# upkie/upkie

Hardware: AMD Instinct MI355X
Metric: env-steps/sec (batched Upkie-Pendulum, 200 Hz) (higher is better)
Workload: dtype f32

## Files before the change

### upkie_amd/csrc/dynamics.hpp

```cpp
#pragma once

#include <hip/hip_runtime.h>

#include "../../include/upkie_hip.h"

#define UPKIE_HD __host__ __device__ __forceinline__

namespace upkie {

UPKIE_HD float fast_rcp(float x) {
#if defined(__HIP_DEVICE_COMPILE__)
  return __builtin_amdgcn_rcpf(x);
#else
  return 1.f / x;
#endif
}
UPKIE_HD float fast_sqrt(float x) {
#if defined(__HIP_DEVICE_COMPILE__)
  return __builtin_amdgcn_sqrtf(x);
#else
  return sqrtf(x);
#endif
}
UPKIE_HD float fast_rsqrt(float x) {
// ... 128 lines not shown
  int enforce_joint_limits;
};

struct DevLimits {
  float lower[UPKIE_NJ];
  float upper[UPKIE_NJ];
  int bounded[UPKIE_NJ];
  int enforce;
};

struct Phys {
  V3 pos;
  float qw, qx, qy, qz;
  V3 linvel;
  V3 angvel;
  float q[UPKIE_NJ];
  float qd[UPKIE_NJ];
};

#if defined(__HIP_DEVICE_COMPILE__)
#define UPKIE_KEEP_IN_SGPR(x) asm volatile("" : "+s"(x))
#else
#define UPKIE_KEEP_IN_SGPR(x) (void)0
#endif

#if defined(__HIP_DEVICE_COMPILE__)
__device__ __forceinline__ void warm_kernel_arguments() {
  auto args = __builtin_amdgcn_kernarg_segment_ptr();
  int sink;
  asm volatile(
      "s_load_dword %0, %1, 0x0\n s_load_dword %0, %1, 0x40\n s_load_dword %0, %1, 0x80\n s_load_dword %0, %1, 0xc0\n"
      "s_load_dword %0, %1, 0x100\n s_load_dword %0, %1, 0x140\n s_load_dword %0, %1, 0x180\n s_load_dword %0, %1, 0x1c0\n"
      "s_load_dword %0, %1, 0x200\n s_load_dword %0, %1, 0x240\n s_load_dword %0, %1, 0x280\n s_load_dword %0, %1, 0x2c0\n"
      "s_load_dword %0, %1, 0x300\n s_load_dword %0, %1, 0x340\n s_load_dword %0, %1, 0x380\n s_load_dword %0, %1, 0x3c0\n"
      "s_load_dword %0, %1, 0x400\n s_load_dword %0, %1, 0x440\n s_load_dword %0, %1, 0x480\n s_load_dword %0, %1, 0x4c0\n"
      "s_waitcnt lgkmcnt(0)"
      : "=&s"(sink)
      : "s"(args)
      : "memory");
}
template <int BYTES, class Ptr>
__device__ __forceinline__ void warm_constant_block(Ptr block) {
  constexpr int LINES = (BYTES + 63) / 64;
  static_assert(LINES <= 24, "block larger than the unrolled touch sequence");
#define UPKIE_LINE(i) "n"(64 * ((i) < LINES ? (i) : LINES - 1))
  int sink;
  asm volatile(
      "s_load_dword %0, %1, %2\n s_load_dword %0, %1, %3\n s_load_dword %0, %1, %4\n s_load_dword %0, %1, %5\n"
      "s_load_dword %0, %1, %6\n s_load_dword %0, %1, %7\n s_load_dword %0, %1, %8\n s_load_dword %0, %1, %9\n"
      "s_load_dword %0, %1, %10\n s_load_dword %0, %1, %11\n s_load_dword %0, %1, %12\n s_load_dword %0, %1, %13\n"
      "s_load_dword %0, %1, %14\n s_load_dword %0, %1, %15\n s_load_dword %0, %1, %16\n s_load_dword %0, %1, %17\n"
      "s_load_dword %0, %1, %18\n s_load_dword %0, %1, %19\n s_load_dword %0, %1, %20\n s_load_dword %0, %1, %21\n"
      "s_load_dword %0, %1, %22\n s_load_dword %0, %1, %23\n s_load_dword %0, %1, %24\n s_load_dword %0, %1, %25\n"
      "s_waitcnt lgkmcnt(0)"
      : "=&s"(sink)
      : "s"(block), UPKIE_LINE(0), UPKIE_LINE(1), UPKIE_LINE(2), UPKIE_LINE(3), UPKIE_LINE(4), UPKIE_LINE(5), UPKIE_LINE(6), UPKIE_LINE(7),
        UPKIE_LINE(8), UPKIE_LINE(9), UPKIE_LINE(10), UPKIE_LINE(11), UPKIE_LINE(12), UPKIE_LINE(13), UPKIE_LINE(14), UPKIE_LINE(15),
        UPKIE_LINE(16), UPKIE_LINE(17), UPKIE_LINE(18), UPKIE_LINE(19), UPKIE_LINE(20), UPKIE_LINE(21), UPKIE_LINE(22), UPKIE_LINE(23)
      : "memory");
#undef UPKIE_LINE
}
#else
__device__ inline void warm_kernel_arguments() {}
template <int BYTES, class Ptr>
__device__ inline void warm_constant_block(Ptr) {}
#endif

struct BaseFrame {
  float r00, r01, r02, r10, r11, r12, r20, r21, r22;
  V3 vB, wB, nB;
};
UPKIE_HD BaseFrame base_frame(float qw, float qx, float qy, float qz, V3 linvel, V3 angvel) {
  BaseFrame f;
  f.r00 = 1.f - 2.f * (qy * qy + qz * qz); f.r01 = 2.f * (qx * qy - qz * qw); f.r02 = 2.f * (qw * qy + qx * qz);
  f.r10 = 2.f * (qx * qy + qz * qw); f.r11 = 1.f - 2.f * (qx * qx + qz * qz); f.r12 = 2.f * (qy * qz - qx * qw);
  f.r20 = 2.f * (qx * qz - qy * qw); f.r21 = 2.f * (qy * qz + qx * qw); f.r22 = 1.f - 2.f * (qx * qx + qy * qy);
  f.vB = v3(f.r00 * linvel.x + f.r10 * linvel.y + f.r20 * linvel.z, f.r01 * linvel.x + f.r11 * linvel.y + f.r21 * linvel.z,
            f.r02 * linvel.x + f.r12 * linvel.y + f.r22 * linvel.z);
  f.wB = v3(f.r00 * angvel.x + f.r10 * angvel.y + f.r20 * angvel.z, f.r01 * angvel.x + f.r11 * angvel.y + f.r21 * angvel.z,
            f.r02 * angvel.x + f.r12 * angvel.y + f.r22 * angvel.z);
  f.nB = v3(f.r20, f.r21, f.r22);
  return f;
}
UPKIE_HD void integrate_base(const BaseFrame& f, float n0, float n1, float n2, float n3, float n4, float n5, float h, V3& pos, float& qw,
                             float& qx, float& qy, float& qz, V3& linvel, V3& angvel) {
  linvel = v3(f.r00 * n0 + f.r01 * n1 + f.r02 * n2, f.r10 * n0 + f.r11 * n1 + f.r12 * n2, f.r20 * n0 + f.r21 * n1 + f.r22 * n2);
  angvel = v3(f.r00 * n3 + f.r01 * n4 + f.r02 * n5, f.r10 * n3 + f.r11 * n4 + f.r12 * n5, f.r20 * n3 + f.r21 * n4 + f.r22 * n5);
  pos = pos + h * linvel;
  const float wn = fast_sqrt(dot(angvel, angvel));
  const float half = 0.5f * h * wn;
  float ch, k;
  if (half < 0.5f) {
    const float x2 = half * half;
    k = 0.5f * h * (1.f + x2 * (-1.f / 6.f + x2 * (1.f / 120.f + x2 * (-1.f / 5040.f + x2 * (1.f / 362880.f)))));
    ch = 1.f + x2 * (-0.5f + x2 * (1.f / 24.f + x2 * (-1.f / 720.f + x2 * (1.f / 40320.f))));
  } else {
    float sh;
    sincosf(half, &sh, &ch);
    k = sh * fast_rcp(wn);
  }
  const float dw = ch, dx = k * angvel.x, dy = k * angvel.y, dz = k * angvel.z;
  const float nw = dw * qw - dx * qx - dy * qy - dz * qz;
  const float nx = dw * qx + dx * qw + dy * qz - dz * qy;
  const float ny = dw * qy - dx * qz + dy * qw + dz * qx;
  const float nz = dw * qz + dx * qy - dy * qx + dz * qw;
  const float inv = fast_rsqrt(nw * nw + nx * nx + ny * ny + nz * nz);
  qw = nw * inv; qx = nx * inv; qy = ny * inv; qz = nz * inv;
}

struct Ldl6 {
  float l10, l20, l21, l30, l31, l32, l40, l41, l42, l43, l50, l51, l52, l53, l54;
  float i0, i1, i2, i3, i4, i5;
};

UPKIE_HD void ldl6_factor(const float (&A)[21], Ldl6& f) {
  float d0 = A[0];
  f.i0 = fast_rcp(d0);
  float a10 = A[1], a20 = A[3], a30 = A[6], a40 = A[10], a50 = A[15];
  f.l10 = a10 * f.i0; f.l20 = a20 * f.i0; f.l30 = a30 * f.i0; f.l40 = a40 * f.i0; f.l50 = a50 * f.i0;
  float d1 = A[2] - f.l10 * a10;
  f.i1 = fast_rcp(d1);
  float a21 = A[4] - f.l20 * a10, a31 = A[7] - f.l30 * a10, a41 = A[11] - f.l40 * a10, a51 = A[16] - f.l50 * a10;
  f.l21 = a21 * f.i1; f.l31 = a31 * f.i1; f.l41 = a41 * f.i1; f.l51 = a51 * f.i1;
  float d2 = A[5] - f.l20 * a20 - f.l21 * a21;
  f.i2 = fast_rcp(d2);
  float a32 = A[8] - f.l30 * a20 - f.l31 * a21, a42 = A[12] - f.l40 * a20 - f.l41 * a21,
        a52 = A[17] - f.l50 * a20 - f.l51 * a21;
  f.l32 = a32 * f.i2; f.l42 = a42 * f.i2; f.l52 = a52 * f.i2;
  float d3 = A[9] - f.l30 * a30 - f.l31 * a31 - f.l32 * a32;
  f.i3 = fast_rcp(d3);
  float a43 = A[13] - f.l40 * a30 - f.l41 * a31 - f.l42 * a32,
        a53 = A[18] - f.l50 * a30 - f.l51 * a31 - f.l52 * a32;
  f.l43 = a43 * f.i3; f.l53 = a53 * f.i3;
  float d4 = A[14] - f.l40 * a40 - f.l41 * a41 - f.l42 * a42 - f.l43 * a43;
  f.i4 = fast_rcp(d4);
  float a54 = A[19] - f.l50 * a40 - f.l51 * a41 - f.l52 * a42 - f.l53 * a43;
  f.l54 = a54 * f.i4;
  float d5 = A[20] - f.l50 * a50 - f.l51 * a51 - f.l52 * a52 - f.l53 * a53 - f.l54 * a54;
  f.i5 = fast_rcp(d5);
}

UPKIE_HD void ldl6_solve(const Ldl6& f, float (&x)[6]) {
  x[1] -= f.l10 * x[0];
  x[2] -= f.l20 * x[0] + f.l21 * x[1];
  x[3] -= f.l30 * x[0] + f.l31 * x[1] + f.l32 * x[2];
  x[4] -= f.l40 * x[0] + f.l41 * x[1] + f.l42 * x[2] + f.l43 * x[3];
  x[5] -= f.l50 * x[0] + f.l51 * x[1] + f.l52 * x[2] + f.l53 * x[3] + f.l54 * x[4];
  x[0] *= f.i0; x[1] *= f.i1; x[2] *= f.i2; x[3] *= f.i3; x[4] *= f.i4; x[5] *= f.i5;
  x[4] -= f.l54 * x[5];
  x[3] -= f.l43 * x[4] + f.l53 * x[5];
  x[2] -= f.l32 * x[3] + f.l42 * x[4] + f.l52 * x[5];
  x[1] -= f.l21 * x[2] + f.l31 * x[3] + f.l41 * x[4] + f.l51 * x[5];
  x[0] -= f.l10 * x[1] + f.l20 * x[2] + f.l30 * x[3] + f.l40 * x[4] + f.l50 * x[5];
}

struct Leg {
  V3 o[3];
  float F[3][6];
  float Hinv[6];
  float D[6][3];
  float bias[3];
  float sgn[3];
};

struct Composite {
  float m;
  V3 h;
  S3 I;
};

struct BodyInertials {
  float m[UPKIE_NB];
  float c[UPKIE_NB][3];
  float I[UPKIE_NB][6];
};
// ... 1353 lines not shown
```

### upkie_amd/csrc/octet.hpp

```cpp
#pragma once

#if !defined(__HIP_DEVICE_COMPILE__)
struct OctHostLane {
  int lane;
  float* slots;
  void (*barrier)(void*);
  void* arg;
};
inline thread_local OctHostLane* g_oct_lane = nullptr;
inline float oct_host_get(float x, int src) {
  OctHostLane* L = g_oct_lane;
  L->slots[L->lane] = x;
  L->barrier(L->arg);
  const float r = L->slots[src];
  L->barrier(L->arg);
  return r;
}
#endif

template <int S0, int S1, int S2, int S3>
UPKIE_HD float oct_qperm(float x) {
#if defined(__HIP_DEVICE_COMPILE__)
  return __builtin_bit_cast(float, __builtin_amdgcn_update_dpp(0, __builtin_bit_cast(int, x), S0 | (S1 << 2) | (S2 << 4) | (S3 << 6), 0xF, 0xF, true));
#else
// ... 306 lines not shown
  L.sg = t[OT_SIGN];
  L.damping = t[OT_DAMPING];
  L.lower = t[OT_LOWER];
  L.upper = t[OT_UPPER];
  L.bounded = t[OT_BOUNDED] != 0.f && Lm.enforce != 0;
  L.effort = t[OT_EFFORT];
  L.velocity = t[OT_VELOCITY];
  L.wj = t[OT_WJ];
  L.w0 = t[OT_W0];
  L.w0_once = t[OT_W0_ONCE];
  L.keep_psi = t[OT_KEEP_PSI];
  L.kl = t[OT_KL];
  L.ka = t[OT_KA];
  float fr = 0.f, cn = 0.f, mn = 0.f;
#pragma unroll
  for (int j = 0; j < UPKIE_NJ; ++j) {
    fr = j == joint ? C.joint_friction[j] : fr;
    cn = j == joint ? C.control_noise[j] : cn;
    mn = j == joint ? C.measurement_noise[j] : mn;
  }
  L.friction = trunk ? 0.f : fr;
  L.control_noise = trunk ? 0.f : cn;
  L.measurement_noise = trunk ? 0.f : mn;
  {
    const float h = C.h, denom = h * M.contact_stiffness + M.contact_damping;
    L.inv_h = fast_rcp(h);
    L.erp = denom > 0.f ? h * M.contact_stiffness * fast_rcp(denom) : 0.2f;
    L.cfm = denom > 0.f ? fast_rcp(denom * h) : 0.f;
  }
  L.total_mass = oct_esum(L.m);
  (void)Lm;
  return L;
}

struct OctPhys {
  V3 pos;
  float qw, qx, qy, qz;
  V3 linvel, angvel;
  float q, qd;
  float lam_prev = 0.f;
  int swept_prev = 0;
  float bl_applied = 0.f;
};

struct Ldl6Planar {
  float l20, l30, l31, l32, l40, l42, l43, l50, l51, l52, l53, l54;
  float i0, i1, i2, i3, i4, i5;
};
UPKIE_HD void ldl6_factor_planar(const float (&A)[21], Ldl6Planar& f) {
  f.i0 = fast_rcp(A[0]);
  const float a20 = A[3], a30 = A[6], a40 = A[10], a50 = A[15];
  f.l20 = a20 * f.i0; f.l30 = a30 * f.i0; f.l40 = a40 * f.i0; f.l50 = a50 * f.i0;
  f.i1 = fast_rcp(A[2]);
  const float a31 = A[7], a51 = A[16];
  f.l31 = a31 * f.i1; f.l51 = a51 * f.i1;
  const float d2 = A[5] - f.l20 * a20;
  f.i2 = fast_rcp(d2);
  const float a32 = A[8] - f.l30 * a20, a42 = A[12] - f.l40 * a20, a52 = A[17] - f.l50 * a20;
  f.l32 = a32 * f.i2; f.l42 = a42 * f.i2; f.l52 = a52 * f.i2;
  const float d3 = A[9] - f.l30 * a30 - f.l31 * a31 - f.l32 * a32;
  f.i3 = fast_rcp(d3);
  const float a43 = A[13] - f.l40 * a30 - f.l42 * a32, a53 = A[18] - f.l50 * a30 - f.l51 * a31 - f.l52 * a32;
  f.l43 = a43 * f.i3; f.l53 = a53 * f.i3;
  const float d4 = A[14] - f.l40 * a40 - f.l42 * a42 - f.l43 * a43;
  f.i4 = fast_rcp(d4);
  const float a54 = A[19] - f.l50 * a40 - f.l52 * a42 - f.l53 * a43;
  f.l54 = a54 * f.i4;
  const float d5 = A[20] - f.l50 * a50 - f.l51 * a51 - f.l52 * a52 - f.l53 * a53 - f.l54 * a54;
  f.i5 = fast_rcp(d5);
}
UPKIE_HD void ldl6_solve_planar(const Ldl6Planar& f, float (&x)[6]) {
  x[2] -= f.l20 * x[0];
  x[3] -= f.l30 * x[0] + f.l31 * x[1] + f.l32 * x[2];
  x[4] -= f.l40 * x[0] + f.l42 * x[2] + f.l43 * x[3];
  x[5] -= f.l50 * x[0] + f.l51 * x[1] + f.l52 * x[2] + f.l53 * x[3] + f.l54 * x[4];
  x[0] *= f.i0; x[1] *= f.i1; x[2] *= f.i2; x[3] *= f.i3; x[4] *= f.i4; x[5] *= f.i5;
  x[4] -= f.l54 * x[5];
  x[3] -= f.l43 * x[4] + f.l53 * x[5];
  x[2] -= f.l32 * x[3] + f.l42 * x[4] + f.l52 * x[5];
  x[1] -= f.l31 * x[3] + f.l51 * x[5];
  x[0] -= f.l20 * x[2] + f.l30 * x[3] + f.l40 * x[4] + f.l50 * x[5];
}

template <int NE>
UPKIE_HD void oct_gauss_jordan(const OctLane& L, float (&D)[3], float (&E)[NE]) {
  {
    const float ip = fast_rcp(oct_qb<1>(D[0]));
    const float f = (1.f - L.e[0]) * (D[0] * ip);
    D[1] -= f * oct_qb<1>(D[1]);
    D[2] -= f * oct_qb<1>(D[2]);
#pragma unroll
    for (int i = 0; i < NE; ++i) E[i] -= f * oct_qb<1>(E[i]);
  }
  {
    const float ip = fast_rcp(oct_qb<2>(D[1]));
    const float f = (1.f - L.e[1]) * (D[1] * ip);
    D[2] -= f * oct_qb<2>(D[2]);
#pragma unroll
    for (int i = 0; i < NE; ++i) E[i] -= f * oct_qb<2>(E[i]);
  }
  {
    const float ip = fast_rcp(oct_qb<3>(D[2]));
    const float f = (1.f - L.e[2]) * (D[2] * ip);
#pragma unroll
    for (int i = 0; i < NE; ++i) E[i] -= f * oct_qb<3>(E[i]);
  }
  const float diag = L.e[0] * D[0] + L.e[1] * D[1] + L.e[2] * D[2] + L.w0;
  const float id = fast_rcp(diag);
#pragma unroll
  for (int i = 0; i < NE; ++i) E[i] *= id;
}

template <int K>
UPKIE_HD float oct_from_joint(float x) { return oct_qb<K + 1>(x); }

template <class ModelT, class LimitsT>
UPKIE_HD void octet_limit_path_registers(const ModelT& M, const LimitsT& Lm_, const OctLane& L, const Ldl6Planar& fac, const float (&Dc)[6], float hv0,
                               float hv1, float hv2, V3 o, V3 Pc, V3 nB, float iun, V3 vB, V3 wB, float dist, bool active,
                               bool active_partner, float q, float qd, float tl, const float (&rt)[6], float cfm, float erp, float ih, float vmax, float h,
                               float (&xb)[6], float& xl) {
  const bool left = L.leg == 0;
  DevLimits Lm;
#pragma unroll
  for (int j = 0; j < UPKIE_NJ; ++j) {
    Lm.lower[j] = Lm_.lower[j];
    Lm.upper[j] = Lm_.upper[j];
    Lm.bounded[j] = Lm_.bounded[j];
  }
  System S;
  S.A.l10 = 0.f; S.A.l20 = fac.l20; S.A.l21 = 0.f; S.A.l30 = fac.l30; S.A.l31 = fac.l31; S.A.l32 = fac.l32;
  S.A.l40 = fac.l40; S.A.l41 = 0.f; S.A.l42 = fac.l42; S.A.l43 = fac.l43;
  S.A.l50 = fac.l50; S.A.l51 = fac.l51; S.A.l52 = fac.l52; S.A.l53 = fac.l53; S.A.l54 = fac.l54;
  S.A.i0 = fac.i0; S.A.i1 = fac.i1; S.A.i2 = fac.i2; S.A.i3 = fac.i3; S.A.i4 = fac.i4; S.A.i5 = fac.i5;
  const float sa = oct_qb<3>(L.sg);
  const V3 t1 = (sa * iun) * v3(nB.z, 0.f, -nB.x);
  const V3 t2 = cross(nB, t1);
  const V3 d = L.e[0] * nB + L.e[1] * t1 + L.e[2] * t2;
  const V3 Pxd = cross(Pc, d);
  const float Jb[6] = {d.x, d.y, d.z, Pxd.x, Pxd.y, Pxd.z};
  const float srz = L.sg * (Pc.z - o.z), srx = L.sg * (Pc.x - o.x);
  const float Jl[3] = {oct_qb<1>(srz) * d.x - oct_qb<1>(srx) * d.z, oct_qb<2>(srz) * d.x - oct_qb<2>(srx) * d.z,
                       oct_qb<3>(srz) * d.x - oct_qb<3>(srx) * d.z};
  float vnow = Jb[0] * vB.x + Jb[1] * vB.y + Jb[2] * vB.z + Jb[3] * wB.x + Jb[4] * wB.y + Jb[5] * wB.z;
  vnow = oct_sumj(vnow, qd, Jl[0], Jl[1], Jl[2]);
  float Jt[6];
  {
    float acc[5] = {Jb[0], Jb[2], Jb[3], Jb[4], Jb[5]};
    const float dc[5] = {Dc[0], Dc[2], Dc[3], Dc[4], Dc[5]};
    oct_sumj_neg5(acc, dc, Jl[0], Jl[1], Jl[2]);
    Jt[0] = acc[0]; Jt[1] = Jb[1]; Jt[2] = acc[1]; Jt[3] = acc[2]; Jt[4] = acc[3]; Jt[5] = acc[4];
  }
  float Jt6[6][6], Jb6[6][6], Jl6[6][3], vn6[6], q6[6], qd6[6], tl6[2][3], d2[2];
  bool act2[2];
  {
    const float hv[3] = {hv0, hv1, hv2};
    const float other_dist = oct_swp(dist);
    d2[0] = left ? dist : other_dist;
    d2[1] = left ? other_dist : dist;
    act2[0] = left ? active : active_partner;
    act2[1] = left ? active_partner : active;
    auto joint = [&](auto kc) {
      constexpr int k = decltype(kc)::value;
      auto both = [&](float x, float& l_, float& r_) {
        const float own = oct_from_joint<k>(x), other = oct_swp(own);
        l_ = left ? own : other;
        r_ = left ? other : own;
      };
#pragma unroll
// ... 359 lines not shown
      const float x = W[r][i], y = W[r][j];
      W[r][i] = Q[w][0] * x + Q[w][1] * y;
      W[r][j] = Q[w][2] * x + Q[w][3] * y;
    }
    const float x = rhs6[i], y = rhs6[j];
    rhs6[i] = Q[w][0] * x + Q[w][1] * y;
    rhs6[j] = Q[w][2] * x + Q[w][3] * y;
  }
  const bool on[2] = {left ? active : active_partner, left ? active_partner : active};
  const float other_applied = oct_swp(applied);
  float lam[6] = {0.f, 0.f, 0.f, 0.f, 0.f, 0.f};
  lam[0] = on[0] ? 0.85f * (left ? applied : other_applied) : 0.f;
  lam[3] = on[1] ? 0.85f * (left ? other_applied : applied) : 0.f;
#if !defined(__HIP_DEVICE_COMPILE__)
  BulletLikeProbe* const probe = L.l == 1 && L.leg == 0 ? g_bullet_like_probe : nullptr;
  if (probe) {
    float* out = probe->system;
    for (int a = 0; a < 6; ++a)
      for (int b = 0; b < 6; ++b) *out++ = W[a][b];
    for (int a = 0; a < 6; ++a) *out++ = rhs6[a];
    for (int a = 0; a < 6; ++a) *out++ = lam[a];
    *out++ = on[0] ? 1.f : 0.f;
    *out++ = on[1] ? 1.f : 0.f;
    probe->sweeps = 0;
  }
#endif
#if !defined(__HIP_DEVICE_COMPILE__)
  if (probe) {
    for (int it = 0; it < M.pgs_iterations; ++it) {
      float before[6];
      for (int a = 0; a < 6; ++a) before[a] = lam[a];
      bullet_like_sweeps6(W, rhs6, lam, on, 0.f, M.friction_mu, 1);
      if (it < 64) {
        float change = 0.f;
        for (int a = 0; a < 6; ++a) {
          change = fmaxf(change, fabsf(lam[a] - before[a]));
          probe->lam[it][a] = lam[a];
        }
        probe->change[it] = change;
        probe->sweeps = it + 1;
      }
    }
  } else
#endif
    bullet_like_sweeps6(W, rhs6, lam, on, 0.f, M.friction_mu, M.pgs_iterations);
  applied = left ? lam[0] : lam[3];
  float out[6];
#pragma unroll
  for (int w = 0; w < 2; ++w) {
    out[3 * w] = lam[3 * w];
    out[3 * w + 1] = Q[w][0] * lam[3 * w + 1] + Q[w][2] * lam[3 * w + 2];
    out[3 * w + 2] = Q[w][1] * lam[3 * w + 1] + Q[w][3] * lam[3 * w + 2];
  }
  const float mine_l = L.l == 1 ? out[0] : (L.l == 2 ? out[1] : out[2]);
  const float mine_r = L.l == 1 ? out[3] : (L.l == 2 ? out[4] : out[5]);
  return left ? mine_l : mine_r;
}

struct OctDefaultScalars {
  static constexpr float gravity = 9.81f, wheel_radius = 0.05f, contact_breaking_threshold = 0.02f, friction_cfm = 0.01f, friction_mu = 1.0f,
                         max_joint_velocity = 100.0f;
};
template <class ModelT>
inline bool oct_model_has_default_scalars(const ModelT& M) {
  typedef OctDefaultScalars D;
  return M.gravity == D::gravity && M.wheel_radius == D::wheel_radius && M.contact_breaking_threshold == D::contact_breaking_threshold &&
         M.friction_cfm == D::friction_cfm && M.friction_mu == D::friction_mu && M.max_joint_velocity == D::max_joint_velocity;
}
#define OCT_HOT(field) (DEFAULT_SCALARS ? OctDefaultScalars::field : M.field)
enum { OCT_NOT_MINE_INFEASIBLE = -3, OCT_NOT_MINE_LIMIT = -1, OCT_NO_CONTACT = 0, OCT_CONTACT = 1 };
struct OctRare {
  int path, sweeps;
};

template <bool LIMITS_IN_REGISTERS = false, bool DEFAULT_SCALARS = false, bool BULLET_LIKE = false, class ModelT, class LimitsT>
UPKIE_HD int physics_substep_octet(const ModelT& M, const LimitsT& Lm, const OctLane& L, OctPhys& s, float tau, float h,
                                   const float* trunk_wrench, LimitWorkspace* ws, OctRare* census = nullptr, float* manifold_out = nullptr,
                                   size_t manifold_stride = 0) {
  bool at_a_stop = false;
  {
#if defined(UPKIE_AB_OLD_LIMITS)
    const bool own_limit = L.bounded && (s.q <= L.lower || s.q >= L.upper);
#else
    const bool own_limit = joint_limit_near(L.bounded, s.q, L.lower, L.upper, joint_limit_reach(s.qd, OCT_HOT(max_joint_velocity), h));
#endif
    if (__builtin_expect(oct_wave_any(own_limit), 0)) at_a_stop = oct_env_any(own_limit);
  }

  const BaseFrame bf = base_frame(s.qw, s.qx, s.qy, s.qz, s.linvel, s.angvel);
  const V3 vB = bf.vB, wB = bf.wB, nB = bf.nB;
  const V3 gn = OCT_HOT(gravity) * nB;

  const float psi = L.keep_psi * oct_chain(L.sg * s.q);
  float sn, cs;
  joint_sincos(psi, &sn, &cs);
  const float pcs = oct_up1(cs), psn = oct_up1(sn);
  const V3 r = v3(pcs * L.p[0] + psn * L.p[2], L.p[1], pcs * L.p[2] - psn * L.p[0]);
  const float sq = L.sg * s.qd;
  float along[4] = {r.x, r.y, r.z, sq};
  oct_chain(along);
  const V3 o = v3(along[0], along[1], along[2]);
  const float S = along[3], Sp = S - sq;
  const V3 wp = v3(wB.x, wB.y + Sp, wB.z);
  const V3 alp = v3(-Sp * wB.z, 0.f, Sp * wB.x);
  const V3 e = cross(alp, r) + cross(wp, cross(wp, r));
  float ao3[3] = {e.x, e.y, e.z};
  oct_chain(ao3);
  const V3 ao = v3(ao3[0], ao3[1], ao3[2]);

  const V3 w = v3(wB.x, wB.y + S, wB.z);
  const V3 al = v3(-S * wB.z, 0.f, S * wB.x);
  const V3 rc = rot_y(cs, sn, v3(L.c[0], L.c[1], L.c[2]));
  const V3 c = o + rc;
  const S3 Ic = rot_y(cs, sn, S3{L.I[0], L.I[1], L.I[2], L.I[3], L.I[4], L.I[5]});
  const V3 ac = ao + cross(al, rc) + cross(w, cross(w, rc));
  const V3 f = L.m * (ac + gn);
  const V3 Iw = mul(Ic, w);
  const V3 N = mul(Ic, al) + cross(w, Iw) + cross(c, f);
  const V3 mc = L.m * c;
  const S3 Ib = shift_to_origin(Ic, L.m, c);
  V3 Fa, Na;
  {
    const V3 vc = vB + cross(w, rc);
    const float vn = fast_sqrt(dot(vc, vc)), wn = fast_sqrt(dot(w, w));
    Fa = (-L.m * (L.kl + L.kl * vn)) * vc;
    Na = (-(L.ka + L.ka * wn)) * Iw + cross(rc, Fa);
    if (trunk_wrench) {
      Fa = Fa + L.w0_once * v3(trunk_wrench[0], trunk_wrench[1], trunk_wrench[2]);
      Na = Na + L.w0_once * v3(trunk_wrench[3], trunk_wrench[4], trunk_wrench[5]);
    }
  }

  float sub[10] = {L.wj * f.x, L.wj * f.z, L.wj * N.y, L.wj * L.m, L.wj * mc.x, L.wj * mc.y, L.wj * mc.z, L.wj * Ib.xy, L.wj * Ib.yy, L.wj * Ib.yz};
  oct_subtree(sub);
  const float fcx = sub[0], fcz = sub[1], Ncy = sub[2], Cm = sub[3];
  const V3 Ch = v3(sub[4], sub[5], sub[6]);
  const float CIxy = sub[7], CIyy = sub[8], CIyz = sub[9];
  const float oxa_x = -L.sg * o.z, oxa_z = L.sg * o.x;
  const float bias = L.sg * Ncy + oxa_x * fcx + oxa_z * fcz;
  float F[6];
  F[0] = Cm * oxa_x + L.sg * Ch.z;
  F[1] = 0.f;
  F[2] = Cm * oxa_z - L.sg * Ch.x;
  F[3] = L.sg * CIxy + Ch.y * oxa_z;
  F[4] = L.sg * CIyy + (Ch.z * oxa_x - Ch.x * oxa_z);
  F[5] = L.sg * CIyz - Ch.y * oxa_x;

  float h1, h2, h3;
  oct_dot3_all(F[4], F[0], F[2], L.sg, oxa_x, oxa_z, h1, h2, h3);
  const float H00 = oct_qb<1>(h1), H01 = oct_qb<1>(h2), H02 = oct_qb<1>(h3), H11 = oct_qb<2>(h2), H12 = oct_qb<2>(h3), H22 = oct_qb<3>(h3);
  const float i00 = fast_rsqrt(H00);
  const float l10 = H01 * i00, l20 = H02 * i00;
  const float i11 = fast_rsqrt(H11 - l10 * l10);
  const float l21 = (H12 - l20 * l10) * i11;
  const float i22 = fast_rsqrt(H22 - l20 * l20 - l21 * l21);
  auto leg_solve = [&](float b0, float b1, float b2, float& x0, float& x1, float& x2) {
    const float y0 = b0 * i00;
    const float y1 = (b1 - l10 * y0) * i11;
    const float y2 = (b2 - l20 * y0 - l21 * y1) * i22;
    x2 = y2 * i22;
    x1 = (y1 - l21 * x2) * i11;
    x0 = (y0 - l10 * x1 - l20 * x2) * i00;
  };
  float hv0, hv1, hv2;
  leg_solve(L.e[0], L.e[1], L.e[2], hv0, hv1, hv2);
  float Dc[6];
  {
    const float f5[5] = {F[0], F[2], F[3], F[4], F[5]};
    float d5[5];
    oct_sumj5(d5, f5, hv0, hv1, hv2);
    Dc[0] = d5[0]; Dc[1] = 0.f; Dc[2] = d5[1]; Dc[3] = d5[2]; Dc[4] = d5[3]; Dc[5] = d5[4];
  }

  Ldl6Planar fac;
  {
    float P[17];
    P[0] = L.m - Dc[0] * F[0];
    P[1] = -Dc[2] * F[0];
    P[2] = L.m - Dc[2] * F[2];
    P[3] = -Dc[3] * F[0];
    P[4] = -mc.z;
    P[5] = mc.y - Dc[3] * F[2];
    P[6] = Ib.xx - Dc[3] * F[3];
    P[7] = mc.z - Dc[4] * F[0];
    P[8] = -mc.x - Dc[4] * F[2];
    P[9] = Ib.xy - Dc[4] * F[3];
    P[10] = Ib.yy - Dc[4] * F[4];
    P[11] = -mc.y - Dc[5] * F[0];
    P[12] = mc.x;
    P[13] = -Dc[5] * F[2];
    P[14] = Ib.xz - Dc[5] * F[3];
    P[15] = Ib.yz - Dc[5] * F[4];
    P[16] = Ib.zz - Dc[5] * F[5];
    oct_esum(P);
    float A[21];
    A[0] = P[0];
    A[1] = 0.f; A[2] = L.total_mass;
    A[3] = P[1]; A[4] = 0.f; A[5] = P[2];
    A[6] = P[3]; A[7] = P[4]; A[8] = P[5]; A[9] = P[6];
    A[10] = P[7]; A[11] = 0.f; A[12] = P[8]; A[13] = P[9]; A[14] = P[10];
    A[15] = P[11]; A[16] = P[12]; A[17] = P[13]; A[18] = P[14]; A[19] = P[15]; A[20] = P[16];
    ldl6_factor_planar(A, fac);
  }

  const float tl = h * (tau - L.damping * s.qd - bias);
  float rt[6];
  rt[0] = h * (Fa.x - f.x) - Dc[0] * tl;
  rt[1] = h * (Fa.y - f.y);
  rt[2] = h * (Fa.z - f.z) - Dc[2] * tl;
  rt[3] = h * (Na.x - N.x) - Dc[3] * tl;
  rt[4] = h * (Na.y - N.y) - Dc[4] * tl;
  rt[5] = h * (Na.z - N.z) - Dc[5] * tl;
  oct_esum(rt);

  const float un = fast_sqrt(nB.x * nB.x + nB.z * nB.z);
  const float iun = fast_rcp(fmaxf(un, 1e-12f));
  const float ih = L.inv_h, erp = L.erp, cfm = L.cfm;
  const V3 ow = v3(oct_qb<3>(o.x), oct_qb<3>(o.y), oct_qb<3>(o.z));
  const V3 center = ow + v3(L.wheel_center[0], L.wheel_center[1], L.wheel_center[2]);
  const V3 Pc = center + OCT_HOT(wheel_radius) * v3(-nB.x * iun, 0.f, -nB.z * iun);
  const float dist = s.pos.z + dot(nB, Pc);
  const bool active = un >= 1e-6f && dist <= OCT_HOT(contact_breaking_threshold);
  const bool active_partner = oct_swp(active ? 1.f : 0.f) != 0.f;
  const bool both = active && active_partner;

  float xb[6];
  float tlc = tl;
  float xl = 0.f;
  int swept_now = 0;
  float lam_now = 0.f;
  if (__builtin_expect(at_a_stop, 0)) {
    if (census) census->path = OCT_NOT_MINE_LIMIT;
    if (LIMITS_IN_REGISTERS && !BULLET_LIKE) {
      octet_limit_path_registers(M, Lm, L, fac, Dc, hv0, hv1, hv2, o, Pc, nB, iun, vB, wB, dist, active, active_partner, s.q, s.qd, tl, rt, cfm,
                                 erp, ih, OCT_HOT(max_joint_velocity), h, xb, xl);
    } else {
      float lim_bias;
      const float lim_sign = joint_limit_row(L.bounded, s.q, L.lower, L.upper, joint_limit_reach(s.qd, OCT_HOT(max_joint_velocity), h), ih, lim_bias);
      if (BULLET_LIKE && !active) s.bl_applied = 0.f;
      octet_limit_path_scratch<BULLET_LIKE>(M, L, fac, Dc, hv0, hv1, hv2, o, Pc, nB, iun, vB, wB, dist, active, active_partner, s.qd, tl, rt, cfm, erp, ih,
                                            lim_sign, lim_bias, xb, xl, ws[oct_env_slot()], &bf, &s.bl_applied);
    }
  } else if (__builtin_expect(active || active_partner, 1)) {
    const float sa = oct_qb<3>(L.sg);
    const V3 t1 = (sa * iun) * v3(nB.z, 0.f, -nB.x);
    const V3 t2 = cross(nB, t1);
    const V3 d = L.e[0] * nB + L.e[1] * t1 + L.e[2] * t2;
    const V3 Pxd = cross(Pc, d);
    float Jb[6] = {d.x, d.y, d.z, Pxd.x, Pxd.y, Pxd.z};
    const float srz = L.sg * (Pc.z - o.z), srx = L.sg * (Pc.x - o.x);
    const float Jl1 = oct_qb<1>(srz) * d.x - oct_qb<1>(srx) * d.z;
    const float Jl2 = oct_qb<2>(srz) * d.x - oct_qb<2>(srx) * d.z;
    const float Jl3 = oct_qb<3>(srz) * d.x - oct_qb<3>(srx) * d.z;
    float vnow = Jb[0] * vB.x + Jb[1] * vB.y + Jb[2] * vB.z + Jb[3] * wB.x + Jb[4] * wB.y + Jb[5] * wB.z;
    vnow = oct_sumj(vnow, s.qd, Jl1, Jl2, Jl3);
    float Y[6];
    {
      float acc[5] = {Jb[0], Jb[2], Jb[3], Jb[4], Jb[5]};
      const float dc[5] = {Dc[0], Dc[2], Dc[3], Dc[4], Dc[5]};
      oct_sumj_neg5(acc, dc, Jl1, Jl2, Jl3);
      Y[0] = acc[0]; Y[1] = Jb[1]; Y[2] = acc[1]; Y[3] = acc[2]; Y[4] = acc[3]; Y[5] = acc[4];
    }
    float Jt[6];
#pragma unroll
    for (int i = 0; i < 6; ++i) {
      Jt[i] = Y[i];
      Y[i] = fmaf(L.w0, rt[i], Y[i]);
    }
    ldl6_solve_planar(fac, Y);
    float K1, K2, K3;
    leg_solve(Jl1, Jl2, Jl3, K1, K2, K3);
    float vf = vnow;
#pragma unroll
    for (int i = 0; i < 6; ++i) vf = fmaf(Y[i], rt[i], vf);
    vf = oct_sumj(vf, tl, K1, K2, K3);
    const float push = dist <= 0.f ? erp * (-dist) * ih : -dist * ih;
    const float rhs = active ? L.e[0] * push - vf : 0.f;
    float Dg[3], X[3];
    {
      const float Jl[3] = {Jl1, Jl2, Jl3}, Kv[3] = {K1, K2, K3};
      oct_rows9(Dg, Jt, Y, Jl, Kv);
    }
    Dg[0] = active ? fmaf(L.e[0], cfm, Dg[0]) : L.e[0];
    Dg[1] = active ? (BULLET_LIKE ? Dg[1] : fmaf(L.e[1], OCT_HOT(friction_cfm), Dg[1])) : L.e[1];
    Dg[2] = active ? (BULLET_LIKE ? Dg[2] : fmaf(L.e[2], OCT_HOT(friction_cfm), Dg[2])) : L.e[2];
    float JtP[6];
#pragma unroll
    for (int i = 0; i < 6; ++i) JtP[i] = oct_swp(Jt[i]);
    oct_rows6(X, JtP, Y);
#pragma unroll
    for (int i = 0; i < 3; ++i) X[i] = both ? X[i] : 0.f;
    float lam;
    if constexpr (BULLET_LIKE) {
      if (!active) s.bl_applied = 0.f;
      lam = oct_bullet_like_solve(M, L, bf, Dg, X, rhs, t1, t2, oct_qb<2>(vf), oct_qb<3>(vf), active, active_partner, s.bl_applied);
    } else {
    {
      float Dw[3] = {Dg[0], Dg[1], Dg[2]};
      float W[4] = {X[0], X[1], X[2], rhs};
      oct_gauss_jordan<4>(L, Dw, W);
      float WP[4];
#pragma unroll
      for (int i = 0; i < 4; ++i) WP[i] = oct_swp(W[i]);
      float Sd[3], rr[1];
      {
        float acc[4] = {Dg[0], Dg[1], Dg[2], rhs};
        oct_sumj_neg4(acc, WP, X[0], X[1], X[2]);
        Sd[0] = acc[0]; Sd[1] = acc[1]; Sd[2] = acc[2]; rr[0] = acc[3];
      }
      oct_gauss_jordan<1>(L, Sd, rr);
      lam = rr[0];
    }
    {
      const float lam_n = oct_qb<1>(lam);
      const bool bad = L.l == 1 ? lam < 0.f : (L.l != 0 && fabsf(lam) > OCT_HOT(friction_mu) * lam_n);
      if (__builtin_expect(oct_wave_any(bad), 0)) {
        if (oct_env_any(bad)) {
          if (census) census->path = OCT_NOT_MINE_INFEASIBLE;
          const float rhs_n = oct_qb<1>(rhs), rhs_n_other = oct_swp(rhs_n);
          if (rhs_n <= 0.f && rhs_n_other <= 0.f) {
            lam = 0.f;
          } else {
          const bool from_previous = s.swept_prev == (both ? 2 : 1);
          const float start = from_previous ? s.lam_prev : lam;
          const int accepted = oct_active_set(L, Dg, X, rhs, start, OCT_HOT(friction_mu), M.pgs_tolerance, lam);
          if (accepted) {
            if (census) census->sweeps = -accepted;
            swept_now = both ? 2 : 1;
          } else {
          const bool left = L.leg == 0;
          float A6[21], rhs6[6], lam6[6];
          oct_gather_system(L, Dg, X, rhs, A6, rhs6);
          {
            const float l1 = oct_qb<1>(start), l2 = oct_qb<2>(start), l3 = oct_qb<3>(start);
            const float q1 = oct_swp(l1), q2 = oct_swp(l2), q3 = oct_swp(l3);
            lam6[0] = left ? l1 : q1; lam6[1] = left ? l2 : q2; lam6[2] = left ? l3 : q3;
            lam6[3] = left ? q1 : l1; lam6[4] = left ? q2 : l2; lam6[5] = left ? q3 : l3;
          }
#pragma unroll
          for (int w = 0; w < 2; ++w) lam6[3 * w] = fmaxf(lam6[3 * w], 0.f);
#pragma unroll
          for (int r = 0; r < 6; ++r) {
            if ((r % 3) == 0) continue;
            const float lim = OCT_HOT(friction_mu) * lam6[3 * (r / 3)];
            lam6[r] = fminf(fmaxf(lam6[r], -lim), lim);
          }
          const int sweeps = contact_pgs6(M, A6, rhs6, lam6);
          if (census) census->sweeps = sweeps;
          const float mine_l = L.l == 1 ? lam6[0] : (L.l == 2 ? lam6[1] : lam6[2]);
          const float mine_r = L.l == 1 ? lam6[3] : (L.l == 2 ? lam6[4] : lam6[5]);
          lam = left ? mine_l : mine_r;
          swept_now = both ? 2 : 1;
          }
          }
        }
      }
    }
    }
    lam_now = lam;
    const float wgt = L.l == 0 ? L.w0_once : lam;
#pragma unroll
    for (int i = 0; i < 6; ++i) xb[i] = wgt * Y[i];
    oct_esum(xb);
    const float JlT1 = srz * nB.x - srx * nB.z, JlT2 = srz * t1.x - srx * t1.z, JlT3 = srz * t2.x - srx * t2.z;
    tlc = oct_sumj(tl, lam, JlT1, JlT2, JlT3);
  } else {
#pragma unroll
    for (int i = 0; i < 6; ++i) xb[i] = rt[i];
    ldl6_solve_planar(fac, xb);
    if (BULLET_LIKE) s.bl_applied = 0.f;
  }

  if (__builtin_expect(!at_a_stop, 1)) {
    xl = oct_sumj(0.f, tlc, hv0, hv1, hv2);
    xl -= Dc[0] * xb[0] + Dc[2] * xb[2] + Dc[3] * xb[3] + Dc[4] * xb[4] + Dc[5] * xb[5];
  }

  {
    const float v = fminf(fmaxf(s.qd + xl, -OCT_HOT(max_joint_velocity)), OCT_HOT(max_joint_velocity));
    s.qd = L.wj * v;
    s.q = fmaf(h, s.qd, s.q);
  }
  s.lam_prev = lam_now;
  s.swept_prev = swept_now;
  if constexpr (BULLET_LIKE) {
    if (manifold_out) {
      float wsn, wcs;
      joint_sincos(oct_qb<3>(oct_chain(L.sg * fmaf(-h, s.qd, s.q))), &wsn, &wcs);
      const V3 local = rot_y(wcs, -wsn, Pc - ow);
      const float x = s.pos.x + bf.r00 * Pc.x + bf.r01 * Pc.y + bf.r02 * Pc.z, y = s.pos.y + bf.r10 * Pc.x + bf.r11 * Pc.y + bf.r12 * Pc.z;
      if (L.l == 1) {
        float* rec = manifold_out + (size_t)(L.leg * 4 * 8) * manifold_stride;
        const float live = active ? 1.f : 0.f;
        rec[0] = live * local.x; rec[manifold_stride] = live * local.y; rec[2 * manifold_stride] = live * local.z;
        rec[3 * manifold_stride] = live * x; rec[4 * manifold_stride] = live * y; rec[5 * manifold_stride] = 0.f;
        rec[6 * manifold_stride] = active ? s.bl_applied : 0.f;
        rec[7 * manifold_stride] = live;
#pragma unroll
        for (int p = 1; p < 4; ++p) rec[(size_t)(8 * p + 7) * manifold_stride] = 0.f;
      }
    }
  }
  const float n0 = vB.x + xb[0], n1 = vB.y + xb[1], n2 = vB.z + xb[2];
  const float n3 = wB.x + xb[3], n4 = wB.y + xb[4], n5 = wB.z + xb[5];
  integrate_base(bf, n0, n1, n2, n3, n4, n5, h, s.pos, s.qw, s.qx, s.qy, s.qz, s.linvel, s.angvel);
  return (active || active_partner) ? OCT_CONTACT : OCT_NO_CONTACT;
}

#if defined(__HIP_DEVICE_COMPILE__) || defined(__HIPCC__)
__device__ __forceinline__ float oct_uniform(float x) {
  return __builtin_bit_cast(float, __builtin_amdgcn_readfirstlane(__builtin_bit_cast(int, x)));
}

#if defined(UPKIE_OCTET_BUFFERED_STATE)
constexpr bool octet_state_through_descriptor(int, bool) { return UPKIE_OCTET_BUFFERED_STATE != 0; }
#else
constexpr bool octet_state_through_descriptor(int mode, bool in_place) { return mode == MODE_PENDULUM_ROLLOUT || in_place; }
#endif

template <class T>
__device__ __forceinline__ T pick6(int j, const T (&a)[6]) {
  return j == 0 ? a[0] : (j == 1 ? a[1] : (j == 2 ? a[2] : (j == 3 ? a[3] : (j == 4 ? a[4] : a[5]))));
}

#if defined(UPKIE_SERVOS_LIMITS_IN_LDS)
constexpr bool kServosLimitsInRegisters = false;
#else
constexpr bool kServosLimitsInRegisters = true;
#endif
#if !defined(UPKIE_PROBE_OCTET_WAVES)
#define UPKIE_PROBE_OCTET_WAVES 2
#endif
#if !defined(UPKIE_OCTET_BLOCK)
#define UPKIE_OCTET_BLOCK 64
#endif
#if defined(UPKIE_STAMPS)
#define UPKIE_STAMP(i) stamp[i] = __builtin_amdgcn_s_memtime()
#define UPKIE_STAMPS_FLUSH()                                                                                                      \
  do {                                                                                                                            \
    UPKIE_STAMP(5);                                                                                            \
    __builtin_amdgcn_s_waitcnt(0);                                                                                                \
    UPKIE_STAMP(6);                                       \
    if (census && (threadIdx.x & 63) == 0) {                                                                                      \
      unsigned long long* out_ = reinterpret_cast<unsigned long long*>(census + UPKIE_CENSUS_WORDS) +                             \
                                 (size_t)8 * (blockIdx.x * (blockDim.x >> 6) + (threadIdx.x >> 6));                               \
      for (int i_ = 0; i_ < 7; ++i_) out_[i_] = stamp[i_];                                                                        \
      out_[7] = __builtin_amdgcn_s_memrealtime();           \
    }                                                                                                                             \
  } while (0)
#else
#define UPKIE_STAMP(i) (void)0
#define UPKIE_STAMPS_FLUSH() (void)0
#endif
template <int MODE, bool RAND, bool DEFAULT_SCALARS = false, bool IN_PLACE = false, bool BULLET_LIKE = false>
__global__ __launch_bounds__(UPKIE_OCTET_BLOCK, MODE == MODE_SERVOS && kServosLimitsInRegisters ? 1 : UPKIE_PROBE_OCTET_WAVES) void step_kernel_octet(const DevModel* __restrict__ Mp, const DevParams* __restrict__ Pp,
                                                         int done_pass, int num_envs, float* __restrict__ state, const float* __restrict__ act,
                                                         float* __restrict__ obs, float* __restrict__ reward,
                                                         uint8_t* __restrict__ terminated, uint8_t* __restrict__ truncated,
                                                         const uint8_t* __restrict__ mask, const float* __restrict__ body_inertials,
                                                         const float* __restrict__ ext_force, int packed, BaseVelocityPtrs bv,
                                                         float* __restrict__ final_obs, int n_steps, unsigned* __restrict__ census,
                                                         ServoPolicyArg<MODE> policy_arg, float* __restrict__ manifold) {
#if defined(UPKIE_STAMPS)
  unsigned long long stamp[8] = {0, 0, 0, 0, 0, 0, 0, 0};
#endif
  UPKIE_STAMP(0);
  const int B = num_envs;
  unsigned block = blockIdx.x;
  if ((gridDim.x & 7u) == 0u) block = (block & 7u) * (gridDim.x >> 3) + (block >> 3);
  const int tid = block * blockDim.x + threadIdx.x;
  const int l = tid & 3, quad = (tid >> 2) & 3, leg = quad >> 1;
  const int e = (tid >> 4) * 2 + (quad & 1);
  const bool in_batch = e < B;
  const bool lead = l == 0 && leg == 0;
  const bool jointed = l != 0;
  const int k = jointed ? l - 1 : 0;
  const int joint = 3 * leg + k;
  constexpr bool BUFFERED = octet_state_through_descriptor(MODE, IN_PLACE);
  const unsigned row_bytes = (unsigned)B * 4u;
  const __amdgpu_buffer_rsrc_t state_rsrc = state_descriptor(state, B);
  float* const st = state + (in_batch ? e : 0);
  const unsigned env_off = (unsigned)(in_batch ? e : 0) * 4u;
  const unsigned joint_off = env_off + (unsigned)joint * row_bytes;
  const unsigned legref_off = env_off + (unsigned)(2 * leg + k) * row_bytes;
#define SWI(w, i, off) state_word<BUFFERED>(state_rsrc, st, (size_t)((w) + (i)) * B, (off), (unsigned)(w) * row_bytes)
#define SW(w) SWI(w, 0, env_off)

  OctPhys s;
// ... 188 lines not shown

  Servo cmd{0.f, 0.f, 0.f, 0.f, 0.f, 0.f};
  float a0 = 0.f, a1 = 0.f;
  unsigned episode = 0;
  if (do_reset) {
    episode = ROLLOUT ? (unsigned)episode_word : (unsigned)SW(UPKIE_S_EPISODE);
    Phys full;
    sample_init_state(C, (unsigned)e, episode, full);
    s.pos = full.pos; s.qw = full.qw; s.qx = full.qx; s.qy = full.qy; s.qz = full.qz;
    s.linvel = full.linvel; s.angvel = full.angvel;
    s.q = jointed ? pick6(joint, full.q) : 0.f;
    s.qd = 0.f;
    s.bl_applied = 0.f;
  } else if (MODE == MODE_SERVOS) {
    if (jointed) {
      float a[6];
      if (policy) {
#pragma unroll
        for (int i = 0; i < 6; ++i) a[i] = policy->action[joint][i];
        float fb = policy->pitch_to_velocity[joint] * policy_pitch + policy->position_to_velocity[joint] * policy_position +
                   policy->velocity_to_velocity[joint] * policy_velocity;
        const float clip = policy->velocity_feedback_clip[joint];
        if (clip > 0.f) fb = fminf(fmaxf(fb, -clip), clip);
        a[1] += fb;
        a[2] += policy->pitch_to_torque[joint] * policy_pitch;
      } else {
        const float* given = act + (size_t)36 * e + 6 * joint;
#pragma unroll
        for (int i = 0; i < 6; ++i) a[i] = given[i];
      }
      const float eff = L.effort, vel = L.velocity;
      cmd.position = clamp_ref(a[0], L.lower, L.upper);
      cmd.velocity = clamp_ref(a[1], -vel, vel);
      cmd.feedforward_torque = clamp_ref(a[2], -eff, eff);
      cmd.kp_scale = clamp_ref(a[3], 0.f, max_gain_scale);
      cmd.kd_scale = clamp_ref(a[4], 0.f, max_gain_scale);
      cmd.maximum_torque = clamp_ref(a[5], 0.f, eff);
#if !defined(UPKIE_AB_NO_GUARD)
      if (const int replaced = guard_servo_command(cmd, eff)) guard_count(C.guard, 0, replaced);
#endif
    }
  } else if (MODE != MODE_RESET) {
    if (fused_agent(MODE)) {
      const float4 o = prev_obs;
      a0 = agent_gain0 * o.x + agent_gain1 * o.y + agent_gain2 * o.z + agent_gain3 * o.w;
      a0 = clamp_ref(a0, -agent_clip, agent_clip);
    } else {
      a0 = act0;
      a1 = act1;
    }
    {
      const int replaced = guard_velocity_actions(a0, a1, max_yaw_velocity);
      if (lead && replaced) guard_count(C.guard, 0, replaced);
    }
    const float v = clamp_ref(a0, -max_ground_velocity, max_ground_velocity);
    const float yawd = clamp_ref(a1, -max_yaw_velocity, max_yaw_velocity);
    const float wheel_velocity = v * inv_radius;
    float left = left_sign * wheel_velocity, right = -left_sign * wheel_velocity;
    left = fmaf(yaw_to_wheel, yawd, left);
    right = fmaf(yaw_to_wheel, yawd, right);
    const float alpha = step_dt / 1.0f;
    legref = legref + alpha * (0.f - legref);
    if (legged) {
      cmd.position = clamp_ref(legref, L.lower, L.upper);
      cmd.kp_scale = clamp_ref(leg_gain_scale, 0.f, max_gain_scale);
      cmd.kd_scale = cmd.kp_scale;
      cmd.maximum_torque = L.effort;
    } else if (l == 3) {
      cmd.position = NAN;
      cmd.velocity = clamp_ref(leg ? right : left, -L.velocity, L.velocity);
      cmd.kp_scale = 1.f;
      cmd.kd_scale = 1.f;
      cmd.maximum_torque = L.effort;
    }
  }

#if defined(UPKIE_STAMPS)
  __builtin_amdgcn_s_waitcnt(0);
#endif
  UPKIE_STAMP(1);
  float tau = 0.f;
  bool contact = false;
  const int nsub = do_reset ? 1 : nb_substeps;
  for (int sub = 0; sub < nb_substeps; ++sub) {
    if (sub >= nsub) break;
    float noise = 0.f;
    if (any_control_noise && !do_reset) {
      float zn[6];
      philox_normal6(C, (unsigned)e, step_count, (unsigned)sub, zn);
      noise = L.control_noise * pick6(joint, zn);
    }
    tau = jointed ? joint_torque(s.q, s.qd, cmd, kp_gain, kd_gain, L.friction, noise) : 0.f;
    ConstModelPtr mp = (ConstModelPtr)Mp;
    asm volatile("" : "+s"(mp));
    const bool forces = RAND && ext.force && !do_reset;
    float wrench[6];
    if (forces) {
      const BaseFrame bf = base_frame(s.qw, s.qx, s.qy, s.qz, s.linvel, s.angvel);
      const float r00 = bf.r00, r01 = bf.r01, r02 = bf.r02, r10 = bf.r10, r11 = bf.r11, r12 = bf.r12, r20 = bf.r20, r21 = bf.r21, r22 = bf.r22;
      V3 Fs = v3(0.f, 0.f, 0.f), Ns = v3(0.f, 0.f, 0.f);
      for (int i = 0; i < C.ext.count; ++i) {
        const V3 f = v3(ext.force[(size_t)(3 * i) * ext.stride], ext.force[(size_t)(3 * i + 1) * ext.stride], ext.force[(size_t)(3 * i + 2) * ext.stride]);
        const V3 pt = v3(C.ext.point[i][0], C.ext.point[i][1], C.ext.point[i][2]);
        const V3 Fe = C.ext.local[i] != 0 ? f : v3(r00 * f.x + r10 * f.y + r20 * f.z, r01 * f.x + r11 * f.y + r21 * f.z, r02 * f.x + r12 * f.y + r22 * f.z);
        Fs = Fs + Fe;
        Ns = Ns + cross(pt, Fe);
      }
      wrench[0] = Fs.x; wrench[1] = Fs.y; wrench[2] = Fs.z; wrench[3] = Ns.x; wrench[4] = Ns.y; wrench[5] = Ns.z;
    }
    OctRare rare_path{0, 0};
    const int status = physics_substep_octet<MODE == MODE_SERVOS && kServosLimitsInRegisters && !BULLET_LIKE, DEFAULT_SCALARS, BULLET_LIKE>(
        *mp, Lm, L, s, tau, substep_h, forces ? wrench : nullptr, limit_ws, &rare_path, BULLET_LIKE && sub == nsub - 1 ? manifold + e : nullptr, (size_t)B);
    const int rare = rare_path.path;
    if (census) {
      const unsigned long long limited = __builtin_amdgcn_ballot_w64(lead && rare == OCT_NOT_MINE_LIMIT);
      const unsigned long long swept = __builtin_amdgcn_ballot_w64(lead && rare == OCT_NOT_MINE_INFEASIBLE);
      const bool first = __builtin_amdgcn_mbcnt_hi(~0u, __builtin_amdgcn_mbcnt_lo(~0u, 0u)) == (unsigned)__builtin_ctzll(__builtin_amdgcn_ballot_w64(true));
      if (first && limited) {
        atomicAdd(&census[0], (unsigned)__builtin_popcountll(limited));
        atomicAdd(&census[4], 1u);
      }
      if (first && swept) atomicAdd(&census[2], (unsigned)__builtin_popcountll(swept));
      if (swept) {
        unsigned total = 0, most = 0, capped = 0, direct = 0;
        for (unsigned long long left = swept; left; left &= left - 1) {
          const int code = __builtin_amdgcn_readlane(rare_path.sweeps, __builtin_ctzll(left));
          const unsigned count = code > 0 ? (unsigned)code : 0u;
          direct += code < 0 ? 1u : 0u;
          total += count;
          most = count > most ? count : most;
          capped += count >= (unsigned)M.pgs_iterations ? 1u : 0u;
        }
        if (first) {
          atomicAdd(&census[6], total);
          if (direct) atomicAdd(&census[3], direct);
          atomicMax(&census[7], most);
          if (capped) atomicAdd(&census[1], capped);
          if (total) {
            atomicAdd(&census[5], 1u);
            atomicAdd(&census[8 + (most < 63u ? most : 63u)], 1u);
          }
        }
      }
    }
    contact = status == OCT_CONTACT;
#if defined(UPKIE_STAMPS)
    if (sub == 0) UPKIE_STAMP(2);
#endif
  }
  UPKIE_STAMP(3);

  bool unsound;
#if defined(UPKIE_AB_NO_GUARD)
  unsound = false;
  if (false)
#endif
  {
    float mag = oct_esum(fabsf(s.q) + fabsf(s.qd));
    mag += fabsf(s.pos.x) + fabsf(s.pos.y) + fabsf(s.pos.z) + fabsf(s.qw) + fabsf(s.qx) + fabsf(s.qy) + fabsf(s.qz);
    mag += fabsf(s.linvel.x) + fabsf(s.linvel.y) + fabsf(s.linvel.z) + fabsf(s.angvel.x) + fabsf(s.angvel.y) + fabsf(s.angvel.z);
    if (YAWING) mag += fabsf(yaw);
    unsound = !(mag < 3.0e38f);
  }
  if (unsound) {
    s.pos = v3(C.init_pos[0], C.init_pos[1], C.init_pos[2]);
    s.qw = C.init_quat[0]; s.qx = C.init_quat[1]; s.qy = C.init_quat[2]; s.qz = C.init_quat[3];
    s.linvel = v3(C.init_linvel[0], C.init_linvel[1], C.init_linvel[2]);
    s.angvel = v3(C.init_angvel[0], C.init_angvel[1], C.init_angvel[2]);
    float init_q[UPKIE_NJ];
#pragma unroll
    for (int j = 0; j < UPKIE_NJ; ++j) init_q[j] = C.init_joint[j];
    s.q = jointed ? pick6(joint, init_q) : 0.f;
    s.qd = 0.f;
    s.bl_applied = 0.f;
    tau = 0.f;
// ... 208 lines not shown
```

Before: 248.8 million.

## Hand-schedule octet Gauss-Jordan in DPP asm and make hot branches wave-uniform

Replaces the NE==4 octet Gauss-Jordan elimination with inline assembly using DPP-fused rcp and fmac to interleave the three pivot steps. It makes the base quaternion integration always evaluate the Taylor series and fall back to sincosf only when some lane in the wave needs it. It also rewrites limit and friction feasibility checks as branchless bit ops, restructures the at_a_stop control flow, gates control-noise generation on a wave-wide ballot, and computes joint torque unconditionally. The aim is to cut divergent branches and instruction count in the hot substep. The hand-written asm depends on DPP hazard nops being correct, which adds risk.

```diff
diff --git a/upkie_amd/csrc/dynamics.hpp b/upkie_amd/csrc/dynamics.hpp
--- a/upkie_amd/csrc/dynamics.hpp
+++ b/upkie_amd/csrc/dynamics.hpp
@@ -234,6 +234,7 @@
   f.nB = v3(f.r20, f.r21, f.r22);
   return f;
 }
+template <bool WAVE_UNIFORM_LIBM = false>
 UPKIE_HD void integrate_base(const BaseFrame& f, float n0, float n1, float n2, float n3, float n4, float n5, float h, V3& pos, float& qw,
                              float& qx, float& qy, float& qz, V3& linvel, V3& angvel) {
   linvel = v3(f.r00 * n0 + f.r01 * n1 + f.r02 * n2, f.r10 * n0 + f.r11 * n1 + f.r12 * n2, f.r20 * n0 + f.r21 * n1 + f.r22 * n2);
@@ -242,7 +243,24 @@
   const float wn = fast_sqrt(dot(angvel, angvel));
   const float half = 0.5f * h * wn;
   float ch, k;
-  if (half < 0.5f) {
+  if constexpr (WAVE_UNIFORM_LIBM) {
+    const float x2 = half * half;
+    k = 0.5f * h * (1.f + x2 * (-1.f / 6.f + x2 * (1.f / 120.f + x2 * (-1.f / 5040.f + x2 * (1.f / 362880.f)))));
+    ch = 1.f + x2 * (-0.5f + x2 * (1.f / 24.f + x2 * (-1.f / 720.f + x2 * (1.f / 40320.f))));
+    const bool beyond = !(half < 0.5f);
+#if defined(__HIP_DEVICE_COMPILE__)
+    const bool some_lane_beyond = __builtin_amdgcn_ballot_w64(beyond) != 0;
+#else
+    const bool some_lane_beyond = beyond;
+#endif
+    if (__builtin_expect(some_lane_beyond, 0)) {
+      if (beyond) {
+        float sh;
+        sincosf(half, &sh, &ch);
+        k = sh * fast_rcp(wn);
+      }
+    }
+  } else if (half < 0.5f) {
     const float x2 = half * half;
     k = 0.5f * h * (1.f + x2 * (-1.f / 6.f + x2 * (1.f / 120.f + x2 * (-1.f / 5040.f + x2 * (1.f / 362880.f)))));
     ch = 1.f + x2 * (-0.5f + x2 * (1.f / 24.f + x2 * (-1.f / 720.f + x2 * (1.f / 40320.f))));
diff --git a/upkie_amd/csrc/octet.hpp b/upkie_amd/csrc/octet.hpp
--- a/upkie_amd/csrc/octet.hpp
+++ b/upkie_amd/csrc/octet.hpp
@@ -412,8 +412,39 @@
   x[0] -= f.l20 * x[2] + f.l30 * x[3] + f.l40 * x[4] + f.l50 * x[5];
 }
 
+#define OCT_GJ(x, f, k) "v_fmac_f32_dpp " x ", -" x ", " f OCT_Q(k)
 template <int NE>
 UPKIE_HD void oct_gauss_jordan(const OctLane& L, float (&D)[3], float (&E)[NE]) {
+#if defined(__HIP_DEVICE_COMPILE__)
+  if constexpr (NE == 4) {
+    const float w1 = 1.f - L.e[0], w2 = 1.f - L.e[1], w3 = 1.f - L.e[2];
+    float ip, iq, f, g;
+    asm("s_nop 1\n\t"
+        "v_rcp_f32_dpp %[ip], %[d0]" OCT_Q(1)
+        "s_nop 0\n\t"
+        "v_mul_f32_e32 %[f], %[d0], %[ip]\n\t"
+        "v_mul_f32_e32 %[f], %[w1], %[f]\n\t"
+        OCT_GJ("%[d1]", "%[f]", 1) OCT_GJ("%[d2]", "%[f]", 1) OCT_GJ("%[e0]", "%[f]", 1)
+        "v_rcp_f32_dpp %[iq], %[d1]" OCT_Q(2)
+        OCT_GJ("%[e1]", "%[f]", 1) OCT_GJ("%[e2]", "%[f]", 1) OCT_GJ("%[e3]", "%[f]", 1)
+        "v_mul_f32_e32 %[g], %[d1], %[iq]\n\t"
+        "v_mul_f32_e32 %[g], %[w2], %[g]\n\t"
+        OCT_GJ("%[d2]", "%[g]", 2) OCT_GJ("%[e0]", "%[g]", 2) OCT_GJ("%[e1]", "%[g]", 2)
+        "v_rcp_f32_dpp %[ip], %[d2]" OCT_Q(3)
+        OCT_GJ("%[e2]", "%[g]", 2) OCT_GJ("%[e3]", "%[g]", 2)
+        "v_mul_f32_e32 %[f], %[d2], %[ip]\n\t"
+        "v_mul_f32_e32 %[f], %[w3], %[f]\n\t"
+        OCT_GJ("%[e0]", "%[f]", 3) OCT_GJ("%[e1]", "%[f]", 3) OCT_GJ("%[e2]", "%[f]", 3) OCT_GJ("%[e3]", "%[f]", 3)
+        : [d1] "+v"(D[1]), [d2] "+v"(D[2]), [e0] "+v"(E[0]), [e1] "+v"(E[1]), [e2] "+v"(E[2]), [e3] "+v"(E[3]), [ip] "=&v"(ip), [iq] "=&v"(iq),
+          [f] "=&v"(f), [g] "=&v"(g)
+        : [d0] "v"(D[0]), [w1] "v"(w1), [w2] "v"(w2), [w3] "v"(w3));
+    const float diag = L.e[0] * D[0] + L.e[1] * D[1] + L.e[2] * D[2] + L.w0;
+    const float id = fast_rcp(diag);
+#pragma unroll
+    for (int i = 0; i < NE; ++i) E[i] *= id;
+    return;
+  }
+#endif
   {
     const float ip = fast_rcp(oct_qb<1>(D[0]));
     const float f = (1.f - L.e[0]) * (D[0] * ip);
@@ -939,7 +970,8 @@
 #if defined(UPKIE_AB_OLD_LIMITS)
     const bool own_limit = L.bounded && (s.q <= L.lower || s.q >= L.upper);
 #else
-    const bool own_limit = joint_limit_near(L.bounded, s.q, L.lower, L.upper, joint_limit_reach(s.qd, OCT_HOT(max_joint_velocity), h));
+    const float zone = joint_limit_reach(s.qd, OCT_HOT(max_joint_velocity), h);
+    const bool own_limit = (int)L.bounded & ((int)(s.q - L.lower <= zone) | (int)(L.upper - s.q <= zone));
 #endif
     if (__builtin_expect(oct_wave_any(own_limit), 0)) at_a_stop = oct_env_any(own_limit);
   }
@@ -1098,7 +1130,9 @@
       octet_limit_path_scratch<BULLET_LIKE>(M, L, fac, Dc, hv0, hv1, hv2, o, Pc, nB, iun, vB, wB, dist, active, active_partner, s.qd, tl, rt, cfm, erp, ih,
                                             lim_sign, lim_bias, xb, xl, ws[oct_env_slot()], &bf, &s.bl_applied);
     }
-  } else if (__builtin_expect(active || active_partner, 1)) {
+  }
+  if (__builtin_expect(!at_a_stop, 1)) {
+  if (__builtin_expect(active || active_partner, 1)) {
     const float sa = oct_qb<3>(L.sg);
     const V3 t1 = (sa * iun) * v3(nB.z, 0.f, -nB.x);
     const V3 t2 = cross(nB, t1);
@@ -1170,7 +1204,7 @@
     }
     {
       const float lam_n = oct_qb<1>(lam);
-      const bool bad = L.l == 1 ? lam < 0.f : (L.l != 0 && fabsf(lam) > OCT_HOT(friction_mu) * lam_n);
+      const bool bad = ((int)(L.l == 1) & (int)(lam < 0.f)) | ((int)(L.l > 1) & (int)(fabsf(lam) > OCT_HOT(friction_mu) * lam_n));
       if (__builtin_expect(oct_wave_any(bad), 0)) {
         if (oct_env_any(bad)) {
           if (census) census->path = OCT_NOT_MINE_INFEASIBLE;
@@ -1228,9 +1262,8 @@
     if (BULLET_LIKE) s.bl_applied = 0.f;
   }
 
-  if (__builtin_expect(!at_a_stop, 1)) {
-    xl = oct_sumj(0.f, tlc, hv0, hv1, hv2);
-    xl -= Dc[0] * xb[0] + Dc[2] * xb[2] + Dc[3] * xb[3] + Dc[4] * xb[4] + Dc[5] * xb[5];
+  xl = oct_sumj(0.f, tlc, hv0, hv1, hv2);
+  xl -= Dc[0] * xb[0] + Dc[2] * xb[2] + Dc[3] * xb[3] + Dc[4] * xb[4] + Dc[5] * xb[5];
   }
 
   {
@@ -1260,7 +1293,7 @@
   }
   const float n0 = vB.x + xb[0], n1 = vB.y + xb[1], n2 = vB.z + xb[2];
   const float n3 = wB.x + xb[3], n4 = wB.y + xb[4], n5 = wB.z + xb[5];
-  integrate_base(bf, n0, n1, n2, n3, n4, n5, h, s.pos, s.qw, s.qx, s.qy, s.qz, s.linvel, s.angvel);
+  integrate_base<true>(bf, n0, n1, n2, n3, n4, n5, h, s.pos, s.qw, s.qx, s.qy, s.qz, s.linvel, s.angvel);
   return (active || active_partner) ? OCT_CONTACT : OCT_NO_CONTACT;
 }
 
@@ -1615,15 +1648,19 @@
   float tau = 0.f;
   bool contact = false;
   const int nsub = do_reset ? 1 : nb_substeps;
+  const bool wave_control_noise = oct_wave_any(any_control_noise && !do_reset);
   for (int sub = 0; sub < nb_substeps; ++sub) {
     if (sub >= nsub) break;
     float noise = 0.f;
-    if (any_control_noise && !do_reset) {
-      float zn[6];
-      philox_normal6(C, (unsigned)e, step_count, (unsigned)sub, zn);
-      noise = L.control_noise * pick6(joint, zn);
-    }
-    tau = jointed ? joint_torque(s.q, s.qd, cmd, kp_gain, kd_gain, L.friction, noise) : 0.f;
+    if (__builtin_expect(wave_control_noise, 0)) {
+      if (any_control_noise && !do_reset) {
+        float zn[6];
+        philox_normal6(C, (unsigned)e, step_count, (unsigned)sub, zn);
+        noise = L.control_noise * pick6(joint, zn);
+      }
+    }
+    const float servo_torque = joint_torque(s.q, s.qd, cmd, kp_gain, kd_gain, L.friction, noise);
+    tau = jointed ? servo_torque : 0.f;
     ConstModelPtr mp = (ConstModelPtr)Mp;
     asm volatile("" : "+s"(mp));
     const bool forces = RAND && ext.force && !do_reset;
```

Measured after the change: 260.3 million (median of 6 runs). 1.05x the previous value.
